# haowenz/chromap

Measured on AMD Instinct MI355X. Metric: M paired reads mapped/s (ATAC preset, GRCh38 index), higher is better.
Workload: dtype u64

## Files before the change

### chromap_amd/csrc/cm_api.hip

```cpp
#include <hip/hip_runtime.h>
#include <math.h>
#include <stdio.h>
#include <stdlib.h>
#include <string.h>

#include <string>
#include <vector>

#include "../../include/chromap_amd.h"
#include "cm_barcode_translate.h"
#include "cm_ctx.h"
#include "cm_kernels.h"
#include "cm_classes.h"
#include "cm_summary.h"
#include "cm_coop.h"
#include <chrono>
#include <mutex>
#include "cm_mapq_tables.h"

static thread_local std::string g_last_error;

static bool cm_debug_pool() { static const bool on = getenv("CM_DEBUG_POOL") != nullptr; return on; }
static thread_local std::string t_last_error;
void cm_set_error(cmgpu_ctx *ctx, const std::string &msg) {
  static std::mutex mu;
  std::lock_guard<std::mutex> lk(mu);
  if (ctx) ctx->err = msg;
  g_last_error = msg;
  t_last_error = msg;
}
extern "C" const char *cmgpu_last_error_thread(void) { return t_last_error.c_str(); }

int DevBuf::ensure(size_t bytes) {
  if (bytes <= cap) return 0;
  if (!owned) return -1;
  static const bool trace = getenv("CM_ALLOC_TRACE") != nullptr;
  const auto t0 = std::chrono::steady_clock::now();
  const size_t had = cap;
// ... 35 lines not shown
    if (value < 0 || value > 4096) { cm_set_error(c, "h2d_copy_blocks: 0..4096"); return CMGPU_EINVAL; }
    c->opt.h2d_kernel = (int)value;
  } else if (n == "d2h_copy_blocks") {
    if (value < 0 || value > 4096) { cm_set_error(c, "d2h_copy_blocks: 0..4096"); return CMGPU_EINVAL; }
    c->opt.d2h_kernel = (int)value;
  } else if (n == "mm_chunks") {
    if (value < 1 || value > CM_MM_CHUNKS) { cm_set_error(c, "mm_chunks: 1.." + std::to_string(CM_MM_CHUNKS)); return CMGPU_EINVAL; }
    c->opt.mm_chunks = (int)value;
  } else if (n == "prep_kernel") {
    c->opt.prep_kernel = (int)value;
  } else if (n == "prep_tile_reads") {
    if (value < 8 || value > 128) { cm_set_error(c, "prep_tile_reads: 8..128"); return CMGPU_EINVAL; }
    c->opt.prep_tile_reads = (int)value;
  } else if (n == "heavy_wave_max" || n == "heavy_block_max" || n == "heavy_big_max") {
    c->opt.heavy_max[n == "heavy_wave_max" ? 0 : n == "heavy_block_max" ? 1 : 2] = (int)value;
  } else if (n == "s3b_lane_cap") {
    if (value < 0 || value > 64) { cm_set_error(c, "s3b_lane_cap: 0 (by read length) or 1..64"); return CMGPU_EINVAL; }
    c->opt.s3b_cap = (int)value;
  } else if (n == "exchange_overlap") {
    c->opt.exchange_overlap = value ? 1 : 0;
  } else if (n == "lanes") {
    if (value < 1 || value > 8) { cm_set_error(c, "lanes: 1..8"); return CMGPU_EINVAL; }
    c->opt.lanes = (int)value;
  } else if (n == "first_read_id") {
    if (value < 0 || value > 0xffffffffll) { cm_set_error(c, "first_read_id: 0..2^32-1"); return CMGPU_EINVAL; }
    c->first_read_id = (uint32_t)value;
  } else if (n == "heavy_mid_max") {
    c->opt.heavy_mid = (int)value;
  } else if (n == "heavy_last") {
    c->opt.heavy_last = (int)value;
  } else if (n == "probe_table_shift") {
    if (value < 0 || value > 4) { cm_set_error(c, "probe_table_shift: 0..4"); return CMGPU_EINVAL; }
    return cm_build_fast_table(c, (int)value);
  } else if (n == "long_read_fused") {
    c->opt.long_fused = value ? 1 : 0;
  } else if (n == "sam_format_group") {
    if (value != 8 && value != 16 && value != 64) { cm_set_error(c, "sam_format_group: 8, 16 or 64"); return CMGPU_EINVAL; }
    c->opt.sam_group = (int)value;
  } else if (n == "verify_planes") {
    c->opt.planes = value ? 1 : 0;
  } else if (n == "speculative_sizes") {
    c->opt.spec = value ? 1 : 0;
    if (value < 0) { c->cls_seen = 0; memset(c->cls_age, 0, sizeof(c->cls_age)); }
  } else if (n == "debug_candidate_capacity") {
    if (value > 0 && cm_ensure_candidate_arrays(c, (uint64_t)value)) { cm_set_error(c, "out of device memory (candidates)"); return CMGPU_ENOMEM; }
    c->pred_m_ok = value > 0; c->m_cap = (uint64_t)value; c->pred_n = 0xffffffffu;
// ... 10 lines not shown
  } else if (n == "generic_kernels") {
    c->opt.generic_kernels = value ? 1 : 0;
  } else if (n == "item_limit") {
    c->opt.item_limit = value > 0 ? (uint64_t)value : 0xfffffff0ull;
  } else {
    cm_set_error(c, "unknown option " + n);
    return CMGPU_EINVAL;
  }
  return CMGPU_OK;
}

extern "C" int cmgpu_get_option(const cmgpu_ctx *c, const char *name, int64_t *value) {
  if (!c || !name || !value) return CMGPU_EINVAL;
  const std::string n(name);
  if (n == "probe_lookups_per_lane") *value = c->opt.probe_variant & 15;
  else if (n == "probe_pair_prefetch") *value = (c->opt.probe_variant & 16) ? 1 : 0;
  else if (n == "mm_chunks") *value = c->opt.mm_chunks;
  else if (n == "h2d_copy_blocks") *value = c->opt.h2d_kernel;
  else if (n == "d2h_copy_blocks") *value = c->opt.d2h_kernel;
  else if (n == "prep_kernel") *value = c->opt.prep_kernel;
  else if (n == "prep_tile_reads") *value = c->opt.prep_tile_reads;
  else if (n == "item_limit") *value = (int64_t)c->opt.item_limit;
  else if (n == "lanes") *value = c->opt.lanes;
  else if (n == "coop") *value = c->opt.coop;
  else if (n == "generic_kernels") *value = c->opt.generic_kernels;
  else if (n == "s3b_short") *value = c->opt.s3b_short;
  else if (n == "pack_once") *value = c->opt.pack_once;
  else if (n == "alloc_us") *value = (int64_t)(c->alloc_seconds * 1e6);
  else if (n == "alloc_draw_us") *value = (int64_t)(c->alloc_draw_seconds * 1e6);
  else if (n.rfind("coop_profile_", 0) == 0) {
    const int k = atoi(n.c_str() + 13);
    unsigned long long v = 0;
    if (k < 0 || k > 63 || !c->coop_prof.p || hipMemcpy(&v, (const unsigned long long *)c->coop_prof.p + k, 8, hipMemcpyDeviceToHost) != hipSuccess) return CMGPU_EINVAL;
    *value = (int64_t)v;
  }
  else if (n == "probe_table_buckets") *value = c->fmask ? (int64_t)c->fmask + 1 : (int64_t)c->bmask + 1;
  else return CMGPU_EINVAL;
  return CMGPU_OK;
}

extern "C" const char *cmgpu_last_error(const cmgpu_ctx *ctx) { return ctx ? ctx->err.c_str() : g_last_error.c_str(); }

__global__ void k_repack(const uint32_t *__restrict__ flags, const uint64_t *__restrict__ keys,
                         const uint64_t *__restrict__ vals, uint64_t *__restrict__ bkt, uint32_t i0, uint32_t n) {
  const uint32_t j = blockIdx.x * 256 + threadIdx.x;
  if (j >= n) return;
// ... 283 lines not shown
extern "C" int cmgpu_set_pairs_chr_order(cmgpu_ctx *c, const uint32_t *rank, uint32_t n) {
  if (!c || !rank) return CMGPU_EINVAL;
  if (n != c->n_seq) { cm_set_error(c, "rank table size differs from the number of reference sequences"); return CMGPU_EINVAL; }
  CM_HIPCHECK(c, cm_enter(c));
  if (c->pairs_rank.ensure((size_t)n * 4)) { cm_set_error(c, "out of device memory (pairs order)"); return CMGPU_ENOMEM; }
  CM_HIPCHECK(c, hipMemcpy(c->pairs_rank.p, rank, (size_t)n * 4, hipMemcpyHostToDevice));
  c->has_pairs_rank = true;
  return CMGPU_OK;
}

extern "C" int cmgpu_destroy(cmgpu_ctx *c) {
  if (!c) return CMGPU_OK;
  if (c->in_flight) { c->worker.join(); c->in_flight = false; }
  for (cmgpu_ctx *l : c->lanes) cmgpu_destroy(l);
  c->lanes.clear();
  if (c->shared_parent) c->shared_parent->shared_children -= 1;
  (void)hipSetDevice(c->device);
  (void)hipDeviceSynchronize();
  cm_exchange_release(c);
  for (DevBuf *b : c->all_bufs()) b->release();
  for (CmFqStream &f : c->fq) if (f.hs) (void)hipStreamDestroy(f.hs);
  for (int i = 0; i < CM_MAX_EVENTS; ++i) if (c->ev[i]) (void)hipEventDestroy(c->ev[i]);
  for (hipEvent_t e : c->chunk_ev) if (e) (void)hipEventDestroy(e);
  if (c->h_maxlen) (void)hipHostFree(c->h_maxlen);
  for (hipEvent_t e : c->ev_h2d) if (e) (void)hipEventDestroy(e);
  if (c->stream_h2d) (void)hipStreamDestroy(c->stream_h2d);
  for (hipEvent_t e : c->ev_d2h) if (e) (void)hipEventDestroy(e);
  if (c->ev_comp) (void)hipEventDestroy(c->ev_comp);
  if (c->stream_d2h) (void)hipStreamDestroy(c->stream_d2h);
  if (c->stream2) (void)hipStreamDestroy(c->stream2);
  if (c->stream_pack) (void)hipStreamDestroy(c->stream_pack);
  if (c->stream) (void)hipStreamDestroy(c->stream);
  delete c;
  return CMGPU_OK;
}

int cm_ensure_slot_scratch(cmgpu_ctx *c, uint64_t slots) {
  if (slots + 1 > 0xffffffffull) { cm_set_error(c, "too many record slots in one batch"); return CMGPU_EINVAL; }
  if (c->scratch_a.ensure((slots + 1) * 4) || c->scratch_b.ensure((slots + 1) * 4) ||
      c->scan_tmp.ensure(cm_scan_tmp_words((uint32_t)slots + 1) * 4)) {
    cm_set_error(c, "out of device memory (record compaction)"); return CMGPU_ENOMEM;
  }
  return CMGPU_OK;
}

static int ensure_pair_arrays(cmgpu_ctx *c, uint32_t n) {
// ... 267 lines not shown
    d.bc_key = c->bc_key.p ? (uint64_t *)c->bc_key.p + lo : nullptr; d.bc_ok = c->bc_ok.p ? (uint8_t *)c->bc_ok.p + lo : nullptr;
  }
}
static inline void mark(cmgpu_ctx *c, const char *name) {
  if (c->n_ev < CM_MAX_EVENTS) {
    (void)hipEventRecord(c->ev[c->n_ev], c->stream);
    c->ev_name[c->n_ev] = name;
    ++c->n_ev;
  }
}
static int scan_with_total(cmgpu_ctx *c, const uint32_t *in, uint32_t *out, uint32_t n, unsigned long long *total, bool wait = true) {
  hipStream_t s = c->stream;
  unsigned long long *acc = (unsigned long long *)c->stats.p + CM_ST_TOTAL;
  CM_HIPCHECK(c, hipMemsetAsync(acc, 0, 8, s));
  cm_launch_k_sum_u32(in, n, acc, s);
  cm_scan_u32(in, out, n, (uint32_t *)c->scan_tmp.p, s);
  CM_HIPCHECK(c, hipMemcpyAsync(total, acc, 8, hipMemcpyDeviceToHost, s));
  if (wait) CM_HIPCHECK(c, cm_stream_sync(s));
  return CMGPU_OK;
}
#define CM_RC_SPLIT (-100)
#define CM_RC_AGAIN_ALL_CLASSES (-101)
#define CM_RC_AGAIN_EXACT_SIZES (-102)
struct RangeRun {
  cmgpu_ctx *c;
  uint32_t rlo, rhi, n, n2;
  bool allow_spec;
  uint64_t limit;
  hipStream_t s;
  CmDev d;
  uint32_t n_mm = 0;
  bool s3a_done = false;
  uint32_t n_heavy[CM_HV_LISTS] = {};
  unsigned long long hits_total = 0;
  uint32_t n_hits = 0;
  bool planes = false;
  bool planes_in_prep = false;
  bool spec = false;
  uint32_t n_m = 0;
  void bind() { cm_bind_dev(c, d, rlo, rhi); }
};
static int stage_begin(RangeRun &r) {
  cmgpu_ctx *c = r.c;
  c->n_ev = 0;
  c->use_perm = false;
  const int rc = ensure_pair_arrays(c, r.n);
  if (rc) return rc;
  CM_HIPCHECK(c, hipMemsetAsync(c->stats.p, 0, CM_ST_N * 8, r.s));
  memset(&r.d, 0, sizeof(r.d));
  cm_ensure_goff(c);
  cm_set_classes(c, r.d);
  r.bind();
  mark(c, "begin");
  if (c->has_barcodes) {
    cm_launch_k_s0b_barcode(r.d, r.n, r.s);
    mark(c, "s0b_barcode");
  }
  return CMGPU_OK;
}
struct MmChunks {
  uint32_t n_chunks;
  uint32_t lo[CM_MM_CHUNKS + 1];
  uint64_t entries[CM_MM_CHUNKS];
  uint32_t part_off[CM_MM_CHUNKS + 1];
};
static uint32_t mm_chunk_count(const RangeRun &r) { return r.n >= (1u << 20) ? (uint32_t)r.c->opt.mm_chunks : (r.n >= (1u << 17) ? 2 : 1); }
static void mm_probe_grids(const cmgpu_ctx *c, MmChunks &k) {
  k.part_off[0] = 0;
  for (uint32_t ch = 0; ch < k.n_chunks; ++ch) k.part_off[ch + 1] = k.part_off[ch] + cm_probe_range_blocks(k.entries[ch], c->opt.probe_variant);
}
template <class Fill>
static int mm_fill_and_probe(RangeRun &r, const MmChunks &k, uint32_t mm_cap, Fill fill) {
  cmgpu_ctx *c = r.c;
  const unsigned long long *marks = (const unsigned long long *)c->mm_marks.p;
  CM_HIPCHECK(c, hipMemsetAsync(r.d.stats + CM_ST_PROBE_STEPS, 0, 2 * 8, r.s));
  for (uint32_t ch = 0; ch < k.n_chunks; ++ch) {
    fill(ch);
    CM_HIPCHECK(c, hipEventRecord(c->chunk_ev[ch], r.s));
    CM_HIPCHECK(c, hipStreamWaitEvent(c->stream2, c->chunk_ev[ch], 0));
    cm_launch_k_probe_range(r.d, marks + ch, k.entries[ch], mm_cap, (uint2 *)c->partials.p + k.part_off[ch], c->stream2, c->opt.probe_variant);
  }
  CM_HIPCHECK(c, hipEventRecord(c->chunk_ev[CM_MM_CHUNKS], c->stream2));
  CM_HIPCHECK(c, hipStreamWaitEvent(r.s, c->chunk_ev[CM_MM_CHUNKS], 0));
  cm_launch_k_probe_reduce(c->partials.p, k.part_off[k.n_chunks], r.d.stats + CM_ST_PROBE_STEPS, r.s);
  return CMGPU_OK;
}
static bool range_wants_planes(const cmgpu_ctx *c) { return c->ref_pl_words != 0 && c->opt.planes; }
static size_t read_planes_bytes(const cmgpu_ctx *c, uint32_t n2) { return (size_t)n2 * cm_read_pl_stride((c->max_read_len + 31) / 32) * 4 + 16; }
static int stage_minimizers_fused(RangeRun &r, bool flat) {
  cmgpu_ctx *c = r.c; CmDev &d = r.d; hipStream_t s = r.s;
  const uint32_t n = r.n, n2 = r.n2;
  int rc;
  const bool pl = !flat && c->opt.pack_once && cm_prep_mm_planes_supported(d, c->max_read_len);
  if (pl && range_wants_planes(c) && !c->read_planes.ensure(read_planes_bytes(c, n2))) {
    d.read_pl = (uint32_t *)c->read_planes.p; d.read_pl_w = (c->max_read_len + 31) / 32;
    r.planes_in_prep = true;
  }
  uint64_t cap = (uint64_t)n2 * (c->max_read_len / 4 + 3);
  const uint64_t bound = (uint64_t)c->bases0 + c->bases1 + 1;
  if (cap > bound) cap = bound;
  const uint32_t ppb = flat ? 128u : cm_prep_mm_pairs_per_block(d, c->max_read_len);
  const uint64_t per_read_bound = c->max_read_len > (uint32_t)c->p.k ? c->max_read_len - (uint32_t)c->p.k + 1 : 1;
  MmChunks k;
  k.n_chunks = mm_chunk_count(r);
  for (int attempt = 0; attempt < 2; ++attempt) {
    if (cap > r.limit) return CM_RC_SPLIT;
    k.lo[0] = 0;
    uint32_t chunk_pairs = 0;
    for (uint32_t ch = 0; ch < k.n_chunks; ++ch) {
      uint64_t hi = (uint64_t)n * (ch + 1) / k.n_chunks;
      hi = ch + 1 == k.n_chunks ? n : hi / ppb * ppb;
      k.lo[ch + 1] = (uint32_t)hi;
      const uint32_t pairs = k.lo[ch + 1] - k.lo[ch];
      chunk_pairs = pairs > chunk_pairs ? pairs : chunk_pairs;
      const uint64_t me = 2ull * pairs * (attempt == 0 ? (uint64_t)(c->max_read_len / 4 + 3) : per_read_bound);
      k.entries[ch] = me > cap ? cap : me;
    }
    mm_probe_grids(c, k);
    if (c->mm_hash.ensure((size_t)cap * 8 + 8) || c->mm_ps.ensure((size_t)cap * 4 + 4) || c->pr_val.ensure((size_t)cap * 8 + 8) ||
        (!flat && c->mm_stage.ensure(cm_prep_mm_stage_bytes(d, c->max_read_len, chunk_pairs) + 8)) ||
        c->pr_kind.ensure((size_t)cap + 4) || c->mm_cursor.ensure(8) || c->mm_marks.ensure((CM_MM_CHUNKS + 1) * 8) ||
        c->partials.ensure(((size_t)k.part_off[k.n_chunks] + 1) * 8 + cm_stats_partial_words(n) * 8)) {
      cm_set_error(c, "out of device memory (minimizers)"); return CMGPU_ENOMEM;
    }
    r.bind();
    CM_HIPCHECK(c, hipMemsetAsync(c->mm_cursor.p, 0, 8, s));
    CM_HIPCHECK(c, hipMemsetAsync(c->mm_marks.p, 0, 8, s));
// ... 8 lines not shown
    CM_HIPCHECK(c, hipMemsetAsync(c->hv_cnt.p, 0, 256, s));
    cm_launch_k_s3a_count(d, n2, s);
    d.mm_cap = 0;
    if ((rc = scan_with_total(c, d.hit_tot, d.hit_off, n2, &r.hits_total, false))) return rc;
    CM_HIPCHECK(c, hipMemcpyAsync(r.n_heavy, c->hv_cnt.p, sizeof(r.n_heavy), hipMemcpyDeviceToHost, s));
    r.s3a_done = true;
    unsigned long long hm[CM_MM_CHUNKS + 1];
    CM_HIPCHECK(c, hipMemcpyAsync(hm, marks, ((size_t)k.n_chunks + 1) * 8, hipMemcpyDeviceToHost, s));
    CM_HIPCHECK(c, cm_stream_sync(s));
    const unsigned long long tot = hm[k.n_chunks];
    bool grid_short = false;
    if (attempt == 0 && tot <= cap)
      for (uint32_t ch = 0; ch < k.n_chunks; ++ch) grid_short = grid_short || hm[ch + 1] - hm[ch] > k.entries[ch];
    if (tot <= cap && !grid_short) { r.n_mm = (uint32_t)tot; break; }
    if (attempt == 1) { cm_set_error(c, "minimizer arrays overflowed twice"); return CMGPU_ECAPACITY; }
    cap = bound;
  }
  mark(c, "s0_s1_s2_trim_minimizers_probe");
  return CMGPU_OK;
}
static int stage_minimizers_two_pass(RangeRun &r) {
  cmgpu_ctx *c = r.c; CmDev &d = r.d; hipStream_t s = r.s;
  int rc;
  cm_launch_k_prep_count(d, r.n, c->max_read_len, s);
  unsigned long long mm_total = 0;
  if ((rc = scan_with_total(c, d.mm_cnt, d.mm_off, r.n2, &mm_total))) return rc;
  if (mm_total > r.limit) return CM_RC_SPLIT;
  const uint32_t n_mm = r.n_mm = (uint32_t)mm_total;
  mark(c, "s0_s1a_trim_count");
  if (c->mm_hash.ensure((size_t)n_mm * 8 + 8) || c->mm_ps.ensure((size_t)n_mm * 4 + 4) || c->pr_val.ensure((size_t)n_mm * 8 + 8) ||
      c->pr_kind.ensure((size_t)n_mm + 4)) { cm_set_error(c, "out of device memory (minimizers)"); return CMGPU_ENOMEM; }
  r.bind();
  MmChunks k;
  k.n_chunks = mm_chunk_count(r);
  for (uint32_t ch = 0; ch <= k.n_chunks; ++ch) k.lo[ch] = (uint32_t)((uint64_t)r.n * ch / k.n_chunks);
  if (c->mm_marks.ensure((CM_MM_CHUNKS + 1) * 8)) { cm_set_error(c, "out of device memory (minimizers)"); return CMGPU_ENOMEM; }
  unsigned long long *marks = (unsigned long long *)c->mm_marks.p;
  unsigned long long hm[CM_MM_CHUNKS + 1];
  cm_launch_k_mm_marks(d.mm_off, k.lo, k.n_chunks + 1, marks, s);
  CM_HIPCHECK(c, hipMemcpyAsync(hm, marks, ((size_t)k.n_chunks + 1) * 8, hipMemcpyDeviceToHost, s));
  CM_HIPCHECK(c, cm_stream_sync(s));
  for (uint32_t ch = 0; ch < k.n_chunks; ++ch) k.entries[ch] = hm[ch + 1] - hm[ch];
  mm_probe_grids(c, k);
  if (c->partials.ensure(((size_t)k.part_off[k.n_chunks] + 1) * 8 + cm_stats_partial_words(r.n) * 8)) { cm_set_error(c, "out of device memory (partials)"); return CMGPU_ENOMEM; }
  if ((rc = mm_fill_and_probe(r, k, n_mm, [&](uint32_t ch) { cm_launch_k_mm_fill(d, k.lo[ch], k.lo[ch + 1], c->max_read_len, s); }))) return rc;
  mark(c, "s1b_s2_minimizers_probe");
// ... 50 lines not shown
  cmgpu_ctx *c = r.c;
  uint64_t waves = (uint64_t)r.n2 / 512 + 64;
  if (waves > 8192) waves = 8192;
  const uint64_t slack = c->rs_pool_want ? waves * CM_POOL_GRANT / 2 : 0;
  uint64_t want = c->rs_pool_want + c->rs_pool_want / 4 + slack;
  if (c->rs_pool_want > c->rs_pool_cap) want = 2 * c->rs_pool_want + slack;
  if (want < (1u << 22)) want = 1u << 22;
  if (want > 0xfffffff0ull) want = 0xfffffff0ull;
  const auto dbg_t0 = std::chrono::steady_clock::now();
  if (c->rs_pool.ensure((size_t)want * 8) == 0 && c->rs_pool_off.ensure((size_t)r.n2 * 2 * 4 + 16) == 0) c->rs_pool_cap = (uint32_t)(c->rs_pool.cap / 8 > 0xfffffff0ull ? 0xfffffff0ull : c->rs_pool.cap / 8);
  else { c->rs_pool.release(); c->rs_pool_cap = 0; }
  if (cm_debug_pool()) fprintf(stderr, "pool ensure want %llu: %.3f ms\n", (unsigned long long)want, std::chrono::duration<double, std::milli>(std::chrono::steady_clock::now() - dbg_t0).count());
  r.bind();
}
static int stage_s4_rescue_filter(RangeRun &r) {
  cmgpu_ctx *c = r.c; CmDev &d = r.d; hipStream_t s = r.s;
  const uint32_t n2 = r.n2;
  const bool coop = (c->opt.coop & 2) != 0;
  CM_HIPCHECK(c, hipMemsetAsync(c->rs_cnt.p, 0, CM_RS_SEGS * 64, s));
  if (coop) size_rescue_pool(r);
  cm_launch_k_s4a_rescue_count(d, n2, s, coop);
  cm_launch_k_s4a_rescue_list(d, n2, s, coop);
  unsigned long long m_total = 0;
  r.spec = r.allow_spec && c->opt.spec && c->pred_m_ok && (c->pred_n == r.n || c->pred_n == 0xffffffffu) && c->m_cap > 0 && c->m_cap <= r.limit;
  if (r.spec) {
    unsigned long long *acc = (unsigned long long *)c->stats.p + CM_ST_TOTAL;
    CM_HIPCHECK(c, hipMemsetAsync(acc, 0, 8, s));
    cm_launch_k_sum_u32(d.m_tot, n2, acc, s);
    cm_scan_u32(d.m_tot, d.m_off, n2, (uint32_t *)c->scan_tmp.p, s);
    cm_launch_k_check_cap(acc, c->m_cap, (unsigned long long *)c->stats.p + CM_ST_ABORT, s);
    r.n_m = (uint32_t)c->m_cap;
  } else {
    const int rc = scan_with_total(c, d.m_tot, d.m_off, n2, &m_total);
    if (rc) return rc;
    if (m_total > r.limit) return CM_RC_SPLIT;
    uint64_t want = m_total + m_total / 4 + 1024;
    if (want > r.limit) want = r.limit;
    if (want < m_total) want = m_total;
    r.n_m = (uint32_t)want;
    if (cm_ensure_candidate_arrays(c, r.n_m)) { cm_set_error(c, "out of device memory (candidates)"); return CMGPU_ENOMEM; }
    c->m_cap = r.n_m;
  }
  if (cm_debug_pool()) fprintf(stderr, "spec %d m_cap %llu m_total %llu\n", (int)r.spec, (unsigned long long)c->m_cap, m_total);
  r.bind();
  mark(c, "s4a_rescue_count");
  cm_launch_k_s4b_rescue_merge(d, n2, s, coop, c->max_read_len);
  cm_launch_k_s4b_rescue_list(d, n2, s, coop, c->max_read_len);
// ... 15 lines not shown
  mark(c, "s5b_verify");
  CM_HIPCHECK(c, hipMemsetAsync(c->srt_cnt.p, 0, 8, s));
  cm_launch_k_s5c_finalize(d, r.n2, s, coop);
  if (c->use_perm) cm_launch_k_sort_lists(d, 1, s);
  mark(c, "s5c_accept");
  return CMGPU_OK;
}
static int stage_s6_records(RangeRun &r) {
  cmgpu_ctx *c = r.c; CmDev &d = r.d; hipStream_t s = r.s;
  const uint32_t n = r.n;
  const bool coop = (c->opt.coop & 16) != 0;
  if (c->p.sam) {
    const uint64_t slots = c->single ? n : r.n2, slot0 = c->single ? r.rlo : 2ull * r.rlo;
    const uint32_t md_cap = c->sam_md_cap;
    const uint32_t zw = (2 * c->p.e + 2 <= 18) ? 5 : 8;
    if (c->sam_z.ensure((size_t)c->max_read_len * zw * 4 * n + 16)) { cm_set_error(c, "out of device memory (SAM buffers)"); return CMGPU_ENOMEM; }
    CM_HIPCHECK(c, hipMemsetAsync((uint8_t *)c->sam_rec.p + slot0 * 40, 0, slots * 40, s));
    d.sam_rec = (uint8_t *)c->sam_rec.p + slot0 * 40; d.sam_cigar = (uint32_t *)c->sam_cigar.p + slot0 * CM_SAM_CIGAR_CAP;
    d.sam_md = (uint8_t *)c->sam_md.p + slot0 * md_cap;
    d.sam_z = (uint32_t *)c->sam_z.p; d.sam_md_cap = md_cap;
  }
  if (c->p.sam) cm_launch_k_s6a_pair_sam(d, n, s); else cm_launch_k_s6a_pair(d, n, s, coop);
  mark(c, "s6a_pairing");
  const uint32_t n_chunks = cm_num_chunks_host(n, (uint32_t)c->p.ref_batch, (uint32_t)c->p.grain);
  cm_launch_k_s6b_sample(d, n_chunks, s);
  if (c->p.sam) cm_launch_k_s6c_multi_sam(d, n, s); else cm_launch_k_s6c_multi(d, n, s, coop);
  mark(c, "s6bc_multimappers");
  return CMGPU_OK;
}
static int stage_finish(RangeRun &r, uint64_t *k_out, cmgpu_stats *stats) {
  cmgpu_ctx *c = r.c; hipStream_t s = r.s;
  cm_launch_k_stats(r.d, r.n, (unsigned long long *)c->partials.p, s);
  unsigned long long hst[CM_ST_N];
  uint32_t h_cls[CM_HV_LISTS];
  CM_HIPCHECK(c, hipMemcpyAsync(hst, c->stats.p, sizeof(hst), hipMemcpyDeviceToHost, s));
  CM_HIPCHECK(c, hipMemcpyAsync(h_cls, c->hv_cnt.p, sizeof(h_cls), hipMemcpyDeviceToHost, s));
  CM_HIPCHECK(c, cm_stream_sync(s));
  mark(c, "stats");
  CM_HIPCHECK(c, cm_stream_sync(s));
  const bool aborted = r.spec && hst[CM_ST_ABORT];
  if (!aborted) {
    unsigned long long seen = 0, keep = 0;
    for (uint32_t l = CM_L_RS_WAVE; l < CM_HV_LISTS; ++l) if (h_cls[l]) seen |= 1ull << (l == CM_L_SEARCH_WAVE_BIG ? CM_L_SEARCH_WAVE : l);
    if (seen & ~r.d.cls_mask) return CM_RC_AGAIN_ALL_CLASSES;
    for (uint32_t l = 0; l < 64; ++l) {
      if ((seen >> l) & 1ull) c->cls_age[l] = 32; else if (c->cls_age[l]) --c->cls_age[l];
      if (c->cls_age[l]) keep |= 1ull << l;
    }
    c->cls_seen = keep;
  } else {
    c->pred_m_ok = false;
    return CM_RC_AGAIN_EXACT_SIZES;
  }
  c->pred_m_ok = true;
  c->pred_n = r.n;
  c->rs_pool_want = hst[CM_ST_POOL];
  if (cm_debug_pool()) fprintf(stderr, "pool: cap %u entries, asked %llu\n", c->rs_pool_cap, (unsigned long long)hst[CM_ST_POOL]);
  if (hst[CM_ST_ERR]) { cm_set_error(c, "internal device error flag " + std::to_string((unsigned long long)hst[CM_ST_ERR])); return CMGPU_ECAPACITY; }
  *k_out = hst[CM_ST_RECORDS];
  c->last_range_lo = r.rlo; c->last_range_hi = r.rhi;
  c->last_n_mm = r.n_mm; c->last_n_hits = r.n_hits; c->last_n_cand_cap = r.n_m;
  if (stats) {
    stats->num_candidates += hst[CM_ST_CAND]; stats->num_mappings += hst[CM_ST_MAPPINGS];
    stats->num_mapped_reads += hst[CM_ST_MAPPED]; stats->num_uniquely_mapped_reads += hst[CM_ST_UNIQ];
    stats->num_minimizers += r.n_mm; stats->probe_steps += hst[CM_ST_PROBE_STEPS]; stats->occurrences_read += hst[CM_ST_OCC];
    stats->num_pairs_rescued += hst[CM_ST_RESCUED]; stats->num_multi_mappers += hst[CM_ST_MULTI];
    stats->num_barcode_in_whitelist += hst[CM_ST_BC_INWL]; stats->num_corrected_barcode += hst[CM_ST_BC_CORR];
  }
  return CMGPU_OK;
}
static int map_range(cmgpu_ctx *c, uint32_t rlo, uint32_t rhi, uint64_t *k_out, cmgpu_stats *stats) {
  bool allow_spec = true;
  int rc;
  *k_out = 0;
  for (;;) {
    RangeRun r = {c, rlo, rhi, rhi - rlo, 2 * (rhi - rlo), allow_spec, c->opt.item_limit, c->stream};
    rc = stage_begin(r);
    if (!rc) {
      const bool flat = c->opt.prep_kernel == 1 && cm_prep_flat_supported(r.d, c->max_read_len, (uint32_t)c->opt.prep_tile_reads);
      const bool fused = flat || (cm_prep_mm_supported(r.d, c->max_read_len) && (c->max_read_len <= 69 || c->opt.long_fused));
      rc = fused ? stage_minimizers_fused(r, flat) : stage_minimizers_two_pass(r);
    }
    if (!rc) rc = stage_pack_reads(r);
    if (!rc) rc = stage_s3_candidates(r);
    if (!rc) rc = stage_s4_rescue_filter(r);
    if (!rc) rc = stage_s5_verify(r);
    if (!rc) rc = stage_s6_records(r);
    if (!rc) rc = stage_finish(r, k_out, stats);
    if (rc == CM_RC_AGAIN_ALL_CLASSES) c->cls_all = true;
    else if (rc == CM_RC_AGAIN_EXACT_SIZES) allow_spec = false;
    else break;
  }
  c->cls_all = false;
  return rc;
}

static int map_split(cmgpu_ctx *c, uint32_t lo, uint32_t hi, uint64_t *k_total, cmgpu_stats *stats) {
  uint64_t k = 0;
  int rc = map_range(c, lo, hi, &k, stats);
  const uint32_t rb = (uint32_t)c->p.ref_batch, n = hi - lo;
  if (rc != CM_RC_SPLIT) { *k_total += k; return rc; }
  if (n <= rb) {
    cm_set_error(c, "a reference batch of " + std::to_string(n) + " pairs needs more than " + std::to_string((unsigned long long)c->opt.item_limit) +
                        " entries in one intermediate array (hits / candidates)");
    return CMGPU_ECAPACITY;
  }
  uint32_t half = (n / 2) / rb * rb;
  if (half == 0) half = rb;
  rc = map_split(c, lo, lo + half, k_total, stats);
  if (rc) return rc;
  return map_split(c, lo + half, hi, k_total, stats);
}

static int lane_prepare(cmgpu_ctx *c, size_t i) {
  while (c->lanes.size() <= i) {
    cmgpu_ctx *l = nullptr;
    const int rc = cmgpu_create_shared(c, &l);
    if (rc) { cm_set_error(c, std::string("lane context: ") + cmgpu_last_error(nullptr)); return rc; }
    c->lanes.push_back(l);
  }
  cmgpu_ctx *l = c->lanes[i];
  auto view = [](DevBuf &dst, const DevBuf &src) { dst.p = src.p; dst.cap = src.cap; dst.owned = false; };
  view(l->bkt_fast, c->bkt_fast); l->fmask = c->fmask;
  view(l->ref_planes, c->ref_planes); l->ref_pl_words = c->ref_pl_words;
  view(l->rb0, c->rb0); view(l->rb1, c->rb1); view(l->ro0, c->ro0); view(l->ro1, c->ro1);
  view(l->rec, c->rec); view(l->rec_ok, c->rec_ok);
  view(l->bcb, c->bcb); view(l->bcq, c->bcq); view(l->bco, c->bco); view(l->bc_key, c->bc_key); view(l->bc_ok, c->bc_ok);
  view(l->wl, c->wl); view(l->pow10_tab, c->pow10_tab);
  view(l->sam_rec, c->sam_rec); view(l->sam_cigar, c->sam_cigar); view(l->sam_md, c->sam_md);
  l->wl_mask = c->wl_mask; l->wl_size = c->wl_size; l->bc_len = c->bc_len; l->wl_num_sample = c->wl_num_sample;
  l->n_pairs = c->n_pairs; l->first_read_id = c->first_read_id; l->bases0 = c->bases0; l->bases1 = c->bases1;
  l->max_read_len = c->max_read_len; l->has_barcodes = c->has_barcodes; l->single = c->single;
  l->sam_slots = c->sam_slots; l->sam_md_cap = c->sam_md_cap;
  l->opt = c->opt;
// ... 16 lines not shown
  if (cm_rec_slots(c) > 0xfffffff0ull) {
    cm_set_error(c, "batch too large: n_pairs * max_num_best_mappings must stay below 2^32");
    return CMGPU_EINVAL;
  }
  if (c->rec.ensure(cm_rec_slots(c) * 24) || c->rec_ok.ensure(cm_rec_slots(c))) { cm_set_error(c, "out of device memory (records)"); return CMGPU_ENOMEM; }
  if (c->has_barcodes && (c->bc_key.ensure((size_t)n * 8) || c->bc_ok.ensure(n))) { cm_set_error(c, "out of device memory (barcodes)"); return CMGPU_ENOMEM; }
  if (c->p.sam) {
    const uint64_t slots = c->single ? n : 2ull * n;
    const uint32_t md_cap = 2 * c->max_read_len + 16;
    if (c->sam_rec.ensure(slots * 40 + 16) || c->sam_cigar.ensure(slots * CM_SAM_CIGAR_CAP * 4 + 16) || c->sam_md.ensure(slots * md_cap + 16)) {
      cm_set_error(c, "out of device memory (SAM buffers)"); return CMGPU_ENOMEM;
    }
    c->sam_slots = slots;
    c->sam_md_cap = md_cap;
  }
  if (c->opt.planes && !c->ref_pl_words && c->ref_bytes) {
    const int rc = cm_build_ref_planes(c);
    if (rc == CMGPU_ENOMEM) {
      c->ref_planes.release(); c->ref_pl_words = 0; c->opt.planes = 0;
      fprintf(stderr, "chromap_amd: no device memory for the reference bit planes, verifying on bytes\n");
    } else if (rc) return rc;
  }
  const uint32_t rb = (uint32_t)c->p.ref_batch;
  uint32_t L = (uint32_t)(c->opt.lanes < 1 ? 1 : c->opt.lanes);
  const uint32_t n_rb = (n + rb - 1) / rb;
  if (L > n_rb) L = n_rb;
  if (n < (1u << 20)) L = 1;
  uint64_t k = 0;
  if (L <= 1) {
    const int rc = map_split(c, 0, n, &k, stats);
    if (rc) return rc;
  } else {
    std::vector<uint32_t> cut(L + 1, 0);
    for (uint32_t i = 1; i < L; ++i) cut[i] = (uint32_t)(((uint64_t)n_rb * i / L) * rb);
    cut[L] = n;
    for (uint32_t i = 1; i < L; ++i) { const int rc = lane_prepare(c, i - 1); if (rc) return rc; }
    std::vector<int> rcs(L, CMGPU_OK);
    std::vector<uint64_t> ks(L, 0);
    std::vector<cmgpu_stats> sts(L);
    for (cmgpu_stats &x : sts) memset(&x, 0, sizeof(x));
    std::vector<std::thread> th;
    for (uint32_t i = 1; i < L; ++i)
      th.emplace_back([&, i]() {
        cmgpu_ctx *l = c->lanes[i - 1];
        (void)hipSetDevice(l->device);
        rcs[i] = map_split(l, cut[i], cut[i + 1], &ks[i], &sts[i]);
      });
    rcs[0] = map_split(c, cut[0], cut[1], &ks[0], &sts[0]);
    for (std::thread &t : th) t.join();
    for (uint32_t i = 0; i < L; ++i) {
      if (rcs[i]) { if (i) cm_set_error(c, c->lanes[i - 1]->err); return rcs[i]; }
      k += ks[i];
      if (stats) {
        uint64_t *dst = reinterpret_cast<uint64_t *>(stats);
        const uint64_t *src = reinterpret_cast<const uint64_t *>(&sts[i]);
        for (size_t q = 0; q < sizeof(cmgpu_stats) / 8; ++q) dst[q] += src[q];
      }
    }
    c->last_range_lo = 0; c->last_range_hi = cut[1];
  }
  c->n_records = k;
  if (n_out) *n_out = k;
  if (c->sm.on) return cm_summary_total(c);
  return CMGPU_OK;
}

static int compact_records(cmgpu_ctx *c, DevBuf &dst) {
  const uint32_t n = (uint32_t)cm_rec_slots(c);
  if (n == 0) return CMGPU_OK;
  { const int rc = cm_ensure_slot_scratch(c, n); if (rc) return rc; }
  if (dst.ensure((size_t)n * 24 + 16)) { cm_set_error(c, "out of device memory (records)"); return CMGPU_ENOMEM; }
  return cm_compact_records(c, dst.p, nullptr, n, c->stream, nullptr);
}
static int download_dense(cmgpu_ctx *c, cmgpu_record *out, uint64_t out_capacity, uint64_t *n_out) {
  if (n_out) *n_out = 0;
  if (cm_rec_slots(c) == 0) return CMGPU_OK;
  if (c->pend_count && c->stream_d2h) CM_HIPCHECK(c, hipStreamSynchronize(c->stream_d2h));
  { const int rc = compact_records(c, c->rec_dense); if (rc) return rc; }
  hipStream_t s = c->stream;
  const uint64_t k = c->n_records;
  if (k > out_capacity) { cm_set_error(c, "record buffer too small"); return CMGPU_ECAPACITY; }
  if (k) { const int rc = device_to_host(c, out, c->rec_dense.p, (size_t)k * 24, s); if (rc) return rc; }
// ... 794 lines not shown
```

### chromap_amd/csrc/cm_ctx.h

```cpp
#ifndef CM_CTX_H_
#define CM_CTX_H_
#include <hip/hip_runtime.h>

#include <string>
#include <thread>
#include <vector>

#include "../../include/chromap_amd.h"
#include "../../include/chromap_amd_debug.h"
#include "cm_types.h"

#define CM_MAX_EVENTS 32
#define CM_MAX_W_HOST 32
#define CM_BZ_SRC_NONE 0
#define CM_BZ_SRC_STORE 1
#define CM_BZ_SRC_UPLOAD 2
#define CM_BZ_SRC_DEVICE 3

struct DevBuf {
  void *p = nullptr;
  size_t cap = 0;
  bool owned = true;
  int ensure(size_t bytes);
  void release();
// ... 63 lines not shown

struct CmExchange {
  int transport = 0;
  int rank = 0, world = 0;
  void *comm = nullptr;
  cmgpu_exchange_transport ext = {};
  std::vector<uint8_t> h_owner;
  DevBuf owner, send, counts , stage;
  unsigned long long *h_matrix = nullptr;
  hipStream_t stream = nullptr;
  hipEvent_t ev_part = nullptr, ev_payload = nullptr;
  bool payload_pending = false;
  uint64_t sent_total = 0, recv_total = 0, steps = 0;
  uint64_t owned_by[64] = {};
};

#define CM_BATCH_SLOTS 8
struct CmBatchSlot {
  DevBuf rb0, rb1, ro0, ro1;
  uint32_t n_pairs = 0, first_read_id = 0, max_read_len = 1;
  size_t bases0 = 0, bases1 = 0;
};

struct CmOptions {
  int long_fused = 1;
  int planes = 1;
  int sam_group = 8;
  int d2h_kernel = 0;
  int h2d_kernel = 0;
  int probe_variant = 1;
  int mm_chunks = CM_MM_CHUNKS;
  int prep_tile_reads = 32;
  int prep_kernel = 0;
  uint64_t item_limit = 0xfffffff0ull;
  int exchange_overlap = 0;
  int s3b_cap = 0;
  int lanes = 1;
  int heavy_mid = 0;
  int heavy_max[3] = {0, 0, 0};
  int heavy_last = 0;
  int spec = 1;
  int pack_once = 1;
  int s3b_short = 1;
  int generic_kernels = 0;
  int coop_rb = 0;
  int coop = 0xff;
};

struct cmgpu_ctx {
  CmOptions opt;
  int device = 0;
  hipStream_t stream = nullptr;
  hipStream_t stream2 = nullptr;
  hipStream_t stream_pack = nullptr;
  hipEvent_t chunk_ev[CM_MM_CHUNKS + 1] = {};
  std::string err;
  cmgpu_params hp;
  CmParams p;
  DevBuf bkt, occ, ref, ref_off, ref_len, len_coef, nsec_break;
  uint32_t bmask = 0, n_occ = 0, n_seq = 0;
  DevBuf bkt_fast, coop_prof;
  uint32_t fmask = 0;
  DevBuf ref_planes, read_planes;
  DevBuf mm_stage;
  uint64_t ref_pl_words = 0;
  int n_break = 0;
  uint64_t ref_bytes = 0;
  std::vector<uint64_t> h_ref_off;
  std::vector<uint32_t> h_ref_len;
  uint32_t n_pairs = 0, first_read_id = 0;
  size_t bases0 = 0, bases1 = 0;
  uint32_t max_read_len = 1;
  DevBuf rb0, rb1, ro0, ro1;
  DevBuf st_rb0, st_rb1, st_ro0, st_ro1, st_bcb, st_bcq, st_bco;
  DevBuf rlen, scratch_a, scratch_b , mm_cnt, mm_off, mm_hash, mm_ps, pr_val, pr_kind;
  DevBuf hit_tot, hit_off, round2, rep_cnt, rep_len, hbuf, hcnt, n_pos_hit, ncp, ncn;
  DevBuf aug, res_neg, res_pos, resc_n, resc_p, m_tot, m_off, mbuf, mcnt, mcp, mcn, force0;
  DevBuf fbuf, fcnt, fcp, fcn, alive, dpos, derr, dsplit, nv, v_off, v_err, v_end, ndp, ndn, min_err, second_err, n_best, n_second;
// ... 163 lines not shown
```

Before: 607.2.

## Add dynamic range planning and staggered front tokens for multi-lane mapping

Replaces the fixed per-lane cut of reads with a planned list of ranges that lanes pull from an atomic counter. A front token can optionally serialize the minimizer/probe front end across lanes using events. Speculative sizing is relaxed so it applies when the batch is no larger than, and at least half of, the previous batch. Default options reproduce the previous cut layout, so most of the new path is opt-in and adds locking and event overhead when enabled.

Result: slower. 595.3 (-2.0%).

```diff
diff --git a/chromap_amd/csrc/cm_api.hip b/chromap_amd/csrc/cm_api.hip
--- a/chromap_amd/csrc/cm_api.hip
+++ b/chromap_amd/csrc/cm_api.hip
@@ -14,6 +14,9 @@
 #include "cm_classes.h"
 #include "cm_summary.h"
 #include "cm_coop.h"
+#include "cm_lane_token.h"
+#include "cm_range_plan.h"
+#include <atomic>
 #include <chrono>
 #include <mutex>
 #include "cm_mapq_tables.h"
@@ -95,6 +98,14 @@
   } else if (n == "lanes") {
     if (value < 1 || value > 8) { cm_set_error(c, "lanes: 1..8"); return CMGPU_EINVAL; }
     c->opt.lanes = (int)value;
+  } else if (n == "range_pairs") {
+    if (value < -1 || value > 0xffffffffll) { cm_set_error(c, "range_pairs: -1, 0 or a pair count"); return CMGPU_EINVAL; }
+    c->opt.range_pairs = value;
+  } else if (n == "lane_stagger") {
+    if (value < 0 || value > 2) { cm_set_error(c, "lane_stagger: 0, 1 or 2"); return CMGPU_EINVAL; }
+    c->opt.lane_stagger = (int)value;
+  } else if (n == "range_cuts") {
+    c->opt.range_cuts = value ? 1 : 0;
   } else if (n == "first_read_id") {
     if (value < 0 || value > 0xffffffffll) { cm_set_error(c, "first_read_id: 0..2^32-1"); return CMGPU_EINVAL; }
     c->first_read_id = (uint32_t)value;
@@ -151,6 +162,9 @@
   else if (n == "prep_tile_reads") *value = c->opt.prep_tile_reads;
   else if (n == "item_limit") *value = (int64_t)c->opt.item_limit;
   else if (n == "lanes") *value = c->opt.lanes;
+  else if (n == "range_pairs") *value = c->opt.range_pairs;
+  else if (n == "lane_stagger") *value = c->opt.lane_stagger;
+  else if (n == "range_cuts") *value = c->opt.range_cuts;
   else if (n == "coop") *value = c->opt.coop;
   else if (n == "generic_kernels") *value = c->opt.generic_kernels;
   else if (n == "s3b_short") *value = c->opt.s3b_short;
@@ -480,6 +494,7 @@
   for (CmFqStream &f : c->fq) if (f.hs) (void)hipStreamDestroy(f.hs);
   for (int i = 0; i < CM_MAX_EVENTS; ++i) if (c->ev[i]) (void)hipEventDestroy(c->ev[i]);
   for (hipEvent_t e : c->chunk_ev) if (e) (void)hipEventDestroy(e);
+  for (hipEvent_t e : c->range_ev) if (e) (void)hipEventDestroy(e);
   if (c->h_maxlen) (void)hipHostFree(c->h_maxlen);
   for (hipEvent_t e : c->ev_h2d) if (e) (void)hipEventDestroy(e);
   if (c->stream_h2d) (void)hipStreamDestroy(c->stream_h2d);
@@ -793,6 +808,15 @@
 #define CM_RC_SPLIT (-100)
 #define CM_RC_AGAIN_ALL_CLASSES (-101)
 #define CM_RC_AGAIN_EXACT_SIZES (-102)
+struct CmRangeTok {
+  CmFrontToken *tok;
+  uint32_t j;
+  hipEvent_t *ev;
+  bool published;
+};
+static void range_tok_give_up(CmRangeTok *t) {
+  if (t && !t->published) { t->published = true; t->tok->publish(t->j, false); }
+}
 struct RangeRun {
   cmgpu_ctx *c;
   uint32_t rlo, rhi, n, n2;
@@ -809,6 +833,7 @@
   bool planes_in_prep = false;
   bool spec = false;
   uint32_t n_m = 0;
+  CmRangeTok *tok = nullptr;
   void bind() { cm_bind_dev(c, d, rlo, rhi); }
 };
 static int stage_begin(RangeRun &r) {
@@ -836,6 +861,11 @@
   uint32_t part_off[CM_MM_CHUNKS + 1];
 };
 static uint32_t mm_chunk_count(const RangeRun &r) { return r.n >= (1u << 20) ? (uint32_t)r.c->opt.mm_chunks : (r.n >= (1u << 17) ? 2 : 1); }
+static int front_token_wait(RangeRun &r) {
+  CmRangeTok *t = r.tok;
+  if (t && t->tok->wait_prev(t->j)) CM_HIPCHECK(r.c, hipStreamWaitEvent(r.s, t->ev[t->j - 1], 0));
+  return CMGPU_OK;
+}
 static void mm_probe_grids(const cmgpu_ctx *c, MmChunks &k) {
   k.part_off[0] = 0;
   for (uint32_t ch = 0; ch < k.n_chunks; ++ch) k.part_off[ch + 1] = k.part_off[ch] + cm_probe_range_blocks(k.entries[ch], c->opt.probe_variant);
@@ -852,6 +882,11 @@
     cm_launch_k_probe_range(r.d, marks + ch, k.entries[ch], mm_cap, (uint2 *)c->partials.p + k.part_off[ch], c->stream2, c->opt.probe_variant);
   }
   CM_HIPCHECK(c, hipEventRecord(c->chunk_ev[CM_MM_CHUNKS], c->stream2));
+  if (r.tok && !r.tok->published) {
+    if (r.tok->tok->awaited(r.tok->j)) CM_HIPCHECK(c, hipEventRecord(r.tok->ev[r.tok->j], c->stream2));
+    r.tok->published = true;
+    r.tok->tok->publish(r.tok->j, true);
+  }
   CM_HIPCHECK(c, hipStreamWaitEvent(r.s, c->chunk_ev[CM_MM_CHUNKS], 0));
   cm_launch_k_probe_reduce(c->partials.p, k.part_off[k.n_chunks], r.d.stats + CM_ST_PROBE_STEPS, r.s);
   return CMGPU_OK;
@@ -874,6 +909,7 @@
   const uint64_t per_read_bound = c->max_read_len > (uint32_t)c->p.k ? c->max_read_len - (uint32_t)c->p.k + 1 : 1;
   MmChunks k;
   k.n_chunks = mm_chunk_count(r);
+  if ((rc = front_token_wait(r))) return rc;
   for (int attempt = 0; attempt < 2; ++attempt) {
     if (cap > r.limit) return CM_RC_SPLIT;
     k.lo[0] = 0;
@@ -928,6 +964,7 @@
 static int stage_minimizers_two_pass(RangeRun &r) {
   cmgpu_ctx *c = r.c; CmDev &d = r.d; hipStream_t s = r.s;
   int rc;
+  if ((rc = front_token_wait(r))) return rc;
   cm_launch_k_prep_count(d, r.n, c->max_read_len, s);
   unsigned long long mm_total = 0;
   if ((rc = scan_with_total(c, d.mm_cnt, d.mm_off, r.n2, &mm_total))) return rc;
@@ -1024,7 +1061,8 @@
   cm_launch_k_s4a_rescue_count(d, n2, s, coop);
   cm_launch_k_s4a_rescue_list(d, n2, s, coop);
   unsigned long long m_total = 0;
-  r.spec = r.allow_spec && c->opt.spec && c->pred_m_ok && (c->pred_n == r.n || c->pred_n == 0xffffffffu) && c->m_cap > 0 && c->m_cap <= r.limit;
+  const bool pred_fits = c->pred_n == 0xffffffffu || (r.n <= c->pred_n && r.n >= c->pred_n / 2);
+  r.spec = r.allow_spec && c->opt.spec && c->pred_m_ok && pred_fits && c->m_cap > 0 && c->m_cap <= r.limit;
   if (r.spec) {
     unsigned long long *acc = (unsigned long long *)c->stats.p + CM_ST_TOTAL;
     CM_HIPCHECK(c, hipMemsetAsync(acc, 0, 8, s));
@@ -1086,8 +1124,15 @@
   }
   if (c->p.sam) cm_launch_k_s6a_pair_sam(d, n, s); else cm_launch_k_s6a_pair(d, n, s, coop);
   mark(c, "s6a_pairing");
-  const uint32_t n_chunks = cm_num_chunks_host(n, (uint32_t)c->p.ref_batch, (uint32_t)c->p.grain);
-  cm_launch_k_s6b_sample(d, n_chunks, s);
+  const uint32_t rb = (uint32_t)c->p.ref_batch;
+  for (const CmRange &pc : cm_range_pieces(r.rlo, r.rhi, rb)) {
+    CmDev dp = d;
+    const uint32_t off = pc.lo - r.rlo;
+    dp.n_pairs = pc.hi - pc.lo;
+    dp.pe_nbest = d.pe_nbest + off;
+    dp.pe_choice = d.pe_choice + (uint64_t)off * (uint32_t)c->p.max_best;
+    cm_launch_k_s6b_sample(dp, cm_num_chunks_host(dp.n_pairs, rb, (uint32_t)c->p.grain), s);
+  }
   if (c->p.sam) cm_launch_k_s6c_multi_sam(d, n, s); else cm_launch_k_s6c_multi(d, n, s, coop);
   mark(c, "s6bc_multimappers");
   return CMGPU_OK;
@@ -1117,7 +1162,7 @@
     return CM_RC_AGAIN_EXACT_SIZES;
   }
   c->pred_m_ok = true;
-  c->pred_n = r.n;
+  if (!r.spec || c->pred_n == 0xffffffffu) c->pred_n = r.n;
   c->rs_pool_want = hst[CM_ST_POOL];
   if (cm_debug_pool()) fprintf(stderr, "pool: cap %u entries, asked %llu\n", c->rs_pool_cap, (unsigned long long)hst[CM_ST_POOL]);
   if (hst[CM_ST_ERR]) { cm_set_error(c, "internal device error flag " + std::to_string((unsigned long long)hst[CM_ST_ERR])); return CMGPU_ECAPACITY; }
@@ -1137,8 +1182,11 @@
   bool allow_spec = true;
   int rc;
   *k_out = 0;
+  CmRangeTok *tok = c->rtok;
+  c->rtok = nullptr;
   for (;;) {
     RangeRun r = {c, rlo, rhi, rhi - rlo, 2 * (rhi - rlo), allow_spec, c->opt.item_limit, c->stream};
+    r.tok = tok;
     rc = stage_begin(r);
     if (!rc) {
       const bool flat = c->opt.prep_kernel == 1 && cm_prep_flat_supported(r.d, c->max_read_len, (uint32_t)c->opt.prep_tile_reads);
@@ -1151,6 +1199,8 @@
     if (!rc) rc = stage_s5_verify(r);
     if (!rc) rc = stage_s6_records(r);
     if (!rc) rc = stage_finish(r, k_out, stats);
+    range_tok_give_up(tok);
+    tok = nullptr;
     if (rc == CM_RC_AGAIN_ALL_CLASSES) c->cls_all = true;
     else if (rc == CM_RC_AGAIN_EXACT_SIZES) allow_spec = false;
     else break;
@@ -1164,16 +1214,15 @@
   int rc = map_range(c, lo, hi, &k, stats);
   const uint32_t rb = (uint32_t)c->p.ref_batch, n = hi - lo;
   if (rc != CM_RC_SPLIT) { *k_total += k; return rc; }
-  if (n <= rb) {
+  const uint32_t mid = cm_split_point(lo, hi, rb);
+  if (mid == 0) {
     cm_set_error(c, "a reference batch of " + std::to_string(n) + " pairs needs more than " + std::to_string((unsigned long long)c->opt.item_limit) +
                         " entries in one intermediate array (hits / candidates)");
     return CMGPU_ECAPACITY;
   }
-  uint32_t half = (n / 2) / rb * rb;
-  if (half == 0) half = rb;
-  rc = map_split(c, lo, lo + half, k_total, stats);
+  rc = map_split(c, lo, mid, k_total, stats);
   if (rc) return rc;
-  return map_split(c, lo + half, hi, k_total, stats);
+  return map_split(c, mid, hi, k_total, stats);
 }
 
 static int lane_prepare(cmgpu_ctx *c, size_t i) {
@@ -1236,31 +1285,50 @@
     } else if (rc) return rc;
   }
   const uint32_t rb = (uint32_t)c->p.ref_batch;
-  uint32_t L = (uint32_t)(c->opt.lanes < 1 ? 1 : c->opt.lanes);
-  const uint32_t n_rb = (n + rb - 1) / rb;
-  if (L > n_rb) L = n_rb;
-  if (n < (1u << 20)) L = 1;
+  const uint32_t lanes = (uint32_t)(c->opt.lanes < 1 ? 1 : c->opt.lanes);
+  std::vector<CmRange> plan;
+  if (lanes > 1 && (n >= (1u << 20) || c->opt.range_pairs > 0)) {
+    const uint64_t target = c->opt.range_pairs >= 0 ? (uint64_t)c->opt.range_pairs : ((uint64_t)n + lanes * CM_RANGES_PER_LANE - 1) / (lanes * CM_RANGES_PER_LANE);
+    plan = cm_plan_ranges(n, rb, (uint32_t)c->p.grain, lanes, target, c->opt.range_cuts != 0);
+  }
+  const uint32_t R = (uint32_t)plan.size(), L = lanes < R ? lanes : R;
   uint64_t k = 0;
   if (L <= 1) {
     const int rc = map_split(c, 0, n, &k, stats);
     if (rc) return rc;
   } else {
-    std::vector<uint32_t> cut(L + 1, 0);
-    for (uint32_t i = 1; i < L; ++i) cut[i] = (uint32_t)(((uint64_t)n_rb * i / L) * rb);
-    cut[L] = n;
     for (uint32_t i = 1; i < L; ++i) { const int rc = lane_prepare(c, i - 1); if (rc) return rc; }
+    while (c->range_ev.size() < R) {
+      hipEvent_t e = nullptr;
+      CM_HIPCHECK(c, hipEventCreateWithFlags(&e, hipEventDisableTiming));
+      c->range_ev.push_back(e);
+    }
+    CmFrontToken token(R, c->opt.lane_stagger, L);
+    std::atomic<uint32_t> next(0);
+    std::atomic<bool> failed(false);
     std::vector<int> rcs(L, CMGPU_OK);
     std::vector<uint64_t> ks(L, 0);
     std::vector<cmgpu_stats> sts(L);
     for (cmgpu_stats &x : sts) memset(&x, 0, sizeof(x));
+    auto run_lane = [&](uint32_t i, cmgpu_ctx *l, uint32_t j) {
+      for (; j < R; j = next.fetch_add(1)) {
+        CmRangeTok rt = {&token, j, c->range_ev.data(), false};
+        l->rtok = &rt;
+        const int rc = failed.load() ? CMGPU_OK : map_split(l, plan[j].lo, plan[j].hi, &ks[i], &sts[i]);
+        l->rtok = nullptr;
+        range_tok_give_up(&rt);
+        if (rc) { rcs[i] = rc; failed.store(true); }
+      }
+    };
+    const uint32_t j0 = next.fetch_add(1);
     std::vector<std::thread> th;
     for (uint32_t i = 1; i < L; ++i)
       th.emplace_back([&, i]() {
         cmgpu_ctx *l = c->lanes[i - 1];
         (void)hipSetDevice(l->device);
-        rcs[i] = map_split(l, cut[i], cut[i + 1], &ks[i], &sts[i]);
+        run_lane(i, l, next.fetch_add(1));
       });
-    rcs[0] = map_split(c, cut[0], cut[1], &ks[0], &sts[0]);
+    run_lane(0, c, j0);
     for (std::thread &t : th) t.join();
     for (uint32_t i = 0; i < L; ++i) {
       if (rcs[i]) { if (i) cm_set_error(c, c->lanes[i - 1]->err); return rcs[i]; }
@@ -1271,7 +1339,6 @@
         for (size_t q = 0; q < sizeof(cmgpu_stats) / 8; ++q) dst[q] += src[q];
       }
     }
-    c->last_range_lo = 0; c->last_range_hi = cut[1];
   }
   c->n_records = k;
   if (n_out) *n_out = k;
diff --git a/chromap_amd/csrc/cm_ctx.h b/chromap_amd/csrc/cm_ctx.h
--- a/chromap_amd/csrc/cm_ctx.h
+++ b/chromap_amd/csrc/cm_ctx.h
@@ -109,6 +109,9 @@
   size_t bases0 = 0, bases1 = 0;
 };
 
+#define CM_RANGES_PER_LANE 1
+#define CM_LANE_STAGGER 0
+#define CM_RANGE_CUTS 1
 struct CmOptions {
   int long_fused = 1;
   int planes = 1;
@@ -130,6 +133,9 @@
   int pack_once = 1;
   int s3b_short = 1;
   int generic_kernels = 0;
+  int64_t range_pairs = -1;
+  int lane_stagger = CM_LANE_STAGGER;
+  int range_cuts = CM_RANGE_CUTS;
   int coop_rb = 0;
   int coop = 0xff;
 };
@@ -141,6 +147,8 @@
   hipStream_t stream2 = nullptr;
   hipStream_t stream_pack = nullptr;
   hipEvent_t chunk_ev[CM_MM_CHUNKS + 1] = {};
+  std::vector<hipEvent_t> range_ev;
+  struct CmRangeTok *rtok = nullptr;
   std::string err;
   cmgpu_params hp;
   CmParams p;
diff --git a/chromap_amd/csrc/cm_lane_token.h b/chromap_amd/csrc/cm_lane_token.h
--- /dev/null
+++ b/chromap_amd/csrc/cm_lane_token.h
@@ -0,0 +1,37 @@
+#ifndef CM_LANE_TOKEN_H_
+#define CM_LANE_TOKEN_H_
+#include <condition_variable>
+#include <cstdint>
+#include <mutex>
+#include <vector>
+
+class CmFrontToken {
+ public:
+  CmFrontToken(uint32_t n_ranges, int stagger, uint32_t lanes) : mode_(stagger), lanes_(lanes), state_(n_ranges, PENDING) {}
+  bool waits(uint32_t j) const { return j > 0 && j < state_.size() && (mode_ == 2 || (mode_ == 1 && j < lanes_)); }
+  bool awaited(uint32_t j) const { return waits(j + 1); }
+  bool wait_prev(uint32_t j) {
+    if (!waits(j)) return false;
+    std::unique_lock<std::mutex> lk(mu_);
+    cv_.wait(lk, [&] { return state_[j - 1] != PENDING; });
+    return state_[j - 1] == RECORDED;
+  }
+  bool publish(uint32_t j, bool recorded) {
+    {
+      std::lock_guard<std::mutex> lk(mu_);
+      if (state_[j] != PENDING) return false;
+      state_[j] = recorded ? RECORDED : GIVEN_UP;
+    }
+    cv_.notify_all();
+    return true;
+  }
+
+ private:
+  enum : uint8_t { PENDING = 0, RECORDED = 1, GIVEN_UP = 2 };
+  const int mode_;
+  const uint32_t lanes_;
+  std::mutex mu_;
+  std::condition_variable cv_;
+  std::vector<uint8_t> state_;
+};
+#endif
diff --git a/chromap_amd/csrc/cm_range_plan.h b/chromap_amd/csrc/cm_range_plan.h
--- /dev/null
+++ b/chromap_amd/csrc/cm_range_plan.h
@@ -0,0 +1,67 @@
+#ifndef CM_RANGE_PLAN_H_
+#define CM_RANGE_PLAN_H_
+#include <algorithm>
+#include <cstdint>
+#include <vector>
+
+struct CmRange { uint32_t lo, hi; };
+
+static inline std::vector<uint32_t> cm_chunk_starts(uint32_t n, uint32_t ref_batch, uint32_t grain) {
+  std::vector<uint32_t> s;
+  for (uint64_t b0 = 0; b0 < n; b0 += ref_batch) {
+    const uint32_t bn = n - b0 < ref_batch ? (uint32_t)(n - b0) : ref_batch;
+    uint32_t T = bn / grain;
+    if (T <= 1) T = 1;
+    const uint32_t dv = bn / T, md = bn % T;
+    for (uint32_t c = 0; c < T; ++c) s.push_back((uint32_t)b0 + c * dv + (c < md ? c : md));
+  }
+  s.push_back(n);
+  return s;
+}
+
+static inline std::vector<CmRange> cm_plan_ranges(uint32_t n, uint32_t ref_batch, uint32_t grain, uint32_t lanes, uint64_t range_pairs, bool rb_cuts) {
+  std::vector<CmRange> out;
+  if (n == 0) return out;
+  if (lanes < 1) lanes = 1;
+  std::vector<uint32_t> cut(1, 0u);
+  if (rb_cuts) {
+    const uint64_t n_rb = ((uint64_t)n + ref_batch - 1) / ref_batch;
+    const uint64_t L = lanes < n_rb ? lanes : n_rb;
+    for (uint64_t i = 1; i < L; ++i) cut.push_back((uint32_t)((n_rb * i / L) * ref_batch));
+  } else {
+    const std::vector<uint32_t> s = cm_chunk_starts(n, ref_batch, grain);
+    const uint64_t target = range_pairs ? range_pairs : ((uint64_t)n + lanes - 1) / lanes;
+    uint64_t R = ((uint64_t)n + target / 2) / target;
+    if (R < 1) R = 1;
+    if (R > s.size() - 1) R = s.size() - 1;
+    for (uint64_t i = 1; i < R; ++i) {
+      const uint64_t ideal = (uint64_t)n * i / R;
+      auto it = std::lower_bound(s.begin(), s.end(), (uint32_t)ideal);
+      uint32_t at = *it;
+      if (it != s.begin() && ideal - *(it - 1) <= (uint64_t)*it - ideal) at = *(it - 1);
+      if (at > cut.back() && at < n) cut.push_back(at);
+    }
+  }
+  cut.push_back(n);
+  for (size_t i = 0; i + 1 < cut.size(); ++i) out.push_back({cut[i], cut[i + 1]});
+  return out;
+}
+
+static inline std::vector<CmRange> cm_range_pieces(uint32_t lo, uint32_t hi, uint32_t ref_batch) {
+  std::vector<CmRange> out;
+  uint64_t a = lo;
+  if (a % ref_batch) {
+    uint64_t b = (a / ref_batch + 1) * ref_batch;
+    if (b > hi) b = hi;
+    out.push_back({(uint32_t)a, (uint32_t)b});
+    a = b;
+  }
+  if (a < hi) out.push_back({(uint32_t)a, hi});
+  return out;
+}
+static inline uint32_t cm_split_point(uint32_t lo, uint32_t hi, uint32_t ref_batch) {
+  uint64_t mid = ((uint64_t)lo + (hi - lo) / 2) / ref_batch * ref_batch;
+  if (mid <= lo) mid = ((uint64_t)lo / ref_batch + 1) * ref_batch;
+  return mid < hi ? (uint32_t)mid : 0u;
+}
+#endif
```
